# Wenyuan-Vincent-Li/Tensorflow-Implementation-of-Triple-GAN

Hardware: AMD Instinct MI355X
Metric: Triple-GAN train images/sec (G+C+D step) CIFAR-10 32x32 bs=100 (higher is better)
Workload: dtype f32; 1 GPU; CIFAR-10 32x32x3, 4000 labelled, bs=100 fp32 (B_G/L_C/U_C/L_D/U_D=100/50/50/20/80), Good_GAN_cifar10 D+G+C step; global_batch=100, parallelism=dp1, exec_mode=auto, exec_mode_chosen=plan, hip_graph=False

## Files before the change

### include/tg_kernels.h

```cpp
#ifndef TG_KERNELS_H
#define TG_KERNELS_H

#include <stdint.h>

#ifdef __cplusplus
extern "C" {
#endif

typedef enum tg_status {
  TG_OK = 0,
  TG_ERR_INVALID = -1,
  TG_ERR_HIP = -2,
  TG_ERR_STATE = -3
} tg_status;

enum { TG_ACT_NONE = 0, TG_ACT_LRELU = 1, TG_ACT_RELU = 2, TG_ACT_TANH = 3, TG_ACT_SIGMOID = 4, TG_ACT_SOFTPLUS = 5 };

int tg_version(void);
const char* tg_last_error_string(void);
int tg_device_count(void);

int tg_graph_begin_capture(void* stream);
int tg_graph_end_capture(void* stream, void** graph_exec_out);
int tg_graph_launch(void* graph_exec, void* stream);
// ... 125 lines not shown
  int64_t tr_sb, tr_st;
  int32_t t, a, b, a_pad, b_pad;
} tg_prep_job;
int tg_filter_prep_multi_f32(const tg_prep_job* jobs, int n_jobs, void* stream);
typedef struct tg_wn_job {
  const float* slab;
  float* dw;
  const float* v;
  const float* g;
  float* dv;
  float* dg;
  float* coef;
  int32_t n_split, t, c_pad, n_pad, c_in, c_out;
} tg_wn_job;
int tg_filter_grad_tail_multi_f32(const tg_wn_job* jobs, int n_jobs, void* stream);
int tg_slab_reduce_f32(const float* slab, int n_split, int t, int c_pad, int n_pad, int c_dim, int n_dim, float* dst, void* stream);

int tg_wn_bwd_f32(const float* dw, const float* v, const float* g, int rows, int c, float* dv, float* dg, float* coef, void* stream);

int64_t tg_colstats_workspace_floats(int rows, int nseg, int c);
int tg_colstats_f32(int mode, const float* a, int ld_a, const float* b, int ld_b, int rows, int c, const int32_t* seg_rows, int nseg, int act,
                    float alpha, float* workspace, float* s1, float* s2, void* stream);
int tg_seg_scale_shift_act_f32(const float* x, int ld_x, float* y, int ld_y, int rows, int c, int c_zero_to, const int32_t* seg_rows, int nseg,
                               const float* scale, const float* shift, int act, float alpha, void* stream);
int64_t tg_wn_init_workspace_floats(int rows, int c);
int tg_wn_init_f32(const float* t, int ld_t, int rows, int c, int c_zero_to, float eps, float init_scale, int act, float alpha,
                   float* workspace, float* g, float* b, float* y, int ld_y, void* stream);
int tg_seg_actgrad_shift_f32(const float* dy, int ld_dy, const float* yact, int ld_y, float* dx, int ld_dx, int rows, int c,
                             const int32_t* seg_rows, int nseg, const float* shift, int act, float alpha, void* stream);
int tg_mobn_finalize_f32(const float* sums, const int32_t* seg_rows, int nseg, int rows, int c, const float* b, float* pop_mean, float decay,
// ... 169 lines not shown
```

### tensorflow-implementation-of-triple-gan_amd/Model/Good_GAN_cifar10.py

```python
import math
import os

import numpy as np

from Model import model_base
from Model import nn
from tg import grad_penalty, ops
from tg.runtime import ParamStore, ctx


def _he_trunc_normal(rng, shape):
    fan_in = shape[-2] * int(np.prod(shape[:-2])) if len(shape) > 2 else shape[0]
    x = rng.standard_normal(shape)
    bad = np.abs(x) > 2
    while bad.any():
        x[bad] = rng.standard_normal(int(bad.sum()))
        bad = np.abs(x) > 2
    return (x * np.sqrt(1.3 * 2.0 / fan_in)).astype(np.float32)


C_CONVS = [
    ('conv1_1', 128, 'SAME', False), ('conv1_2', 128, 'SAME', False), ('conv1_3', 128, 'SAME', True),
    ('conv2_1', 256, 'SAME', False), ('conv2_2', 256, 'SAME', False), ('conv2_3', 256, 'SAME', True), ('conv3', 512, 'VALID', False)]
D_CONVS = [
# ... 191 lines not shown
        with cx.rng_scoped(cx.phase + '/D'):
            dp, dl = self.discriminator(ximg, yall)
        n_p = x_l_d.n + x_u_d.n
        cut = lambda a: [a.view_rows(0, n_p), a.view_rows(n_p, n_p + G.n), a.view_rows(n_p + G.n, a.n)]
        (p_real, p_fake, p_unl), (l_real, l_fake, l_unl) = cut(dp), cut(dl)
        return [G, [p_real, l_real, p_fake, l_fake, p_unl, l_unl], [C_real, C_unl, C_unl_d, C_fake, C_rep]]


def _dense_view(a):
    assert a.ld == a.c, "layer width must be a multiple of 32 here"
    return a


def _onehot_act(logits, k):
    from tg.runtime import Act
    return Act(ops.argmax_onehot(logits, k), logits.n, 1, 1, k, k)



ZCA_EPS = 1e-5
ZCA_DATA = ('cifar10', 'cifar100')
ZCA_CHUNK = 16384
ZCA_N_MAX = math.isqrt((2 ** 63 - 1) >> 14)


def zca_prefix(config):
    return "cifar100" if getattr(config, 'DATA_NAME', None) == "cifar100" else "cifar10"


def zca_paths(config):
    pre = os.path.join(config.DATA_DIR, zca_prefix(config))
# ... 153 lines not shown
```

### tensorflow-implementation-of-triple-gan_amd/Model/nn.py

```python
import numpy as np

from tg import ops
from tg.runtime import ctx


def int_shape(x):
    return [x.n, x.h, x.w, x.c] if (x.h, x.w) != (1, 1) else [x.n, x.c]


def get_name(layer_name, counters):
    if layer_name not in counters:
        counters[layer_name] = 0
    name = layer_name + '_' + str(counters[layer_name])
    counters[layer_name] += 1
    return name


def _normal(std, seed_key):
    def init(shape):
        cx = ctx()
        cx.init_rng = getattr(cx, 'init_rng', None) or np.random.default_rng(20190430)
        return (cx.init_rng.standard_normal(shape) * std).astype(np.float32)
    return init

# ... 58 lines not shown
    g = cx.get_variable('g', (num_out,), 1.0) if use_weight_normalization else None
    trains = cx.trains()
    gr = (lambda leaf: cx.var_grad(leaf)) if trains else (lambda leaf: None)
    a = _tg_act(nonlinearity)
    fuse = dict(act=a[0], alpha=a[1]) if a else {}
    if use_weight_normalization and init and cx.assign_init:
        return _data_init(cx, x, V, g, b, num_out, k, stride, pad, init_eps, init_scale, nonlinearity)
    if use_weight_normalization and init:
        ones = cx.ws('const:ones', max(num_out, 1024))
        ops.fill(ones, 1.0)
        with cx.no_record():
            y = ops.conv2d(x, V, None, num_out, k, stride, pad, wn=(ones, None))
            y = ops.moments_normalize(y, init_eps, init_scale)
            return _apply_nonlinearity(y, nonlinearity)
    if use_weight_normalization and use_mean_only_batch_normalization:
        if a is None and nonlinearity is not None:
            y = ops.conv2d(x, V, None, num_out, k, stride, pad, wn=(g, gr('g')), mobn=(b, gr('b'), pop), segments=segments,
                           train=not deterministic, kernel_grad=gr('V'))
            return nonlinearity(y)
        return ops.conv2d(x, V, None, num_out, k, stride, pad, wn=(g, gr('g')), mobn=(b, gr('b'), pop), segments=segments,
                          train=not deterministic, kernel_grad=gr('V'), pool=then_pool, **fuse)
    if use_weight_normalization:
        y = ops.conv2d(x, V, b, num_out, k, stride, pad, wn=(g, gr('g')), kernel_grad=gr('V'), bias_grad=gr('b'), **fuse)
        return y if (a or nonlinearity is None) else nonlinearity(y)
    if use_batch_normalization:
        y = ops.conv2d(x, V, None, num_out, k, stride, pad, kernel_grad=gr('V'))
        y = batch_norm_impl(y, is_conv_out=k > 1, deterministic=deterministic)
        return _apply_nonlinearity(y, nonlinearity)
    y = ops.conv2d(x, V, b, num_out, k, stride, pad, kernel_grad=gr('V'), bias_grad=gr('b'), **fuse)
    return y if (a or nonlinearity is None) else nonlinearity(y)
# ... 88 lines not shown
```

### tensorflow-implementation-of-triple-gan_amd/Training/Train_goodGAN.py

```python
import contextlib
import math
import os
import time

import numpy as np
import torch

from config import Config
from Training.options import (LOSSES, NETS, NUM_CLASSES_RANGE, OPTIMIZERS, check_act_dtype, check_clip_norm, check_eval_ema, check_loss,
                              check_mfma_dtype, check_num_classes, check_optimizer, check_sample_metrics, check_wn_init, check_zca, cla_lr, opt, resolve)
from Training.train_base import Train_base, clip_workspace_floats
from tg import dist as tgdist
from tg import executor, lib, ops
from tg.batching import concat_acts
from tg.runtime import Act, Context, PhiloxRNG, ctx, set_context


class Train(Train_base):
    def __init__(self, config, log_dir, save_dir, **kwargs):
        super(Train, self).__init__()
        self.config = config
        self.save_dir = save_dir
        self.log_dir = log_dir
        self.comments = kwargs.get('comments', '')
        o = self.options = resolve(config)
        self.world, self.rank, self.local_rank = tgdist.init()
        try:
            self.cx = ctx()
# ... 125 lines not shown
            g_replay = []
            wgan = self.loss_kind == 'WGAN_GP'
            with cx.wgrad_on_side():
                with cx.sub_tape(('good_generator',), replay=g_replay) as g_tape:
                    G = m.good_generator(self.z_g_ph, self.y_g_ph)
                if wgan:
                    xp = concat_acts([m.as_image(self.x_l_d_ph), m.as_image(self.x_u_d_ph)])
                    self._gp_w, self._gp_grad = m.discriminator_gradient_penalty(xp, m.as_image(G), self.y_g_ph, self.GP_WEIGHT, in_step=True)
            self._g_saved = (G, g_tape, g_replay)
            xz = concat_acts([m.as_image(self.x_u_c_ph), m.as_image(self.x_u_d_ph)])
            if m.zca() is not None:
                xz = m.zca().apply(xz)
            with cx.rng_scoped('D/C'):
                c_logits, _ = m.classifier(xz, True, segments=[c.BATCH_SIZE_U_C, c.BATCH_SIZE_U_D])
            cx.join_wgrad_side()
            oh = ops.argmax_onehot(c_logits, c.NUM_CLASSES)
            self._d_logits = c_logits
            if self._label_override.get('D') is not None:
                oh.copy_(self._label_override['D'])
            k = c.NUM_CLASSES
            oh_unl = Act(oh[:c.BATCH_SIZE_U_C * k], c.BATCH_SIZE_U_C, 1, 1, k, k)
            oh_unl_d = Act(oh[c.BATCH_SIZE_U_C * k:], c.BATCH_SIZE_U_D, 1, 1, k, k)
            self._d_labels = (oh_unl, oh_unl_d)
            ximg = concat_acts([m.as_image(a) for a in (self.x_l_d_ph, self.x_u_d_ph, G, self.x_u_c_ph)])
            yall = concat_acts([self.y_l_d_ph, oh_unl_d, self.y_g_ph, oh_unl])
            with cx.rng_scoped('D/D'):
                _, d_logits = m.discriminator(ximg, yall, want_prob=False)
            if wgan:
                self._wgan_d_head(d_logits, c.BATCH_SIZE_L_D + c.BATCH_SIZE_U_D, c.BATCH_SIZE_G, c.BATCH_SIZE_U_C, self.hyper[2:4], self._gp_w,
                                  self.loss_dev[0:1])
            else:
# ... 29 lines not shown
            G = m.good_generator(self.z_g_ph, self.y_g_ph)
            parts = [self.x_l_c_ph, self.x_u_c_ph] + ([self.x_u_c_ph] if rep else []) + [G]
            segs = [p.n for p in parts]
            xc = concat_acts([m.as_image(p) for p in parts])
            if m.zca() is not None:
                xc = m.zca().apply(xc)
            with cx.rng_scoped('C/C'):
                c_logits, _ = m.classifier(xc, True, segments=segs)
            c_unl = c_logits.view_rows(segs[0], segs[0] + segs[1])
            if self.loss_kind == 'WGAN_GP':
                self._c_logits = c_unl
                self._wgan_c_head(c_logits, segs[0], sum(segs[1:-1]), G.n, self.y_l_c_ph, self.y_g_ph, self.hyper[2:4], self.loss_dev[2:3])
                self._keep_rest('C', cx.backward(stop_at_boundary='classifier' if split else False))
                return
            k = c.NUM_CLASSES
            oh_c = ops.argmax_onehot(c_unl, k)
            self._c_logits = c_unl
            if self._label_override.get('C') is not None:
                oh_c.copy_(self._label_override['C'])
            oh_unl = Act(oh_c, c_unl.n, 1, 1, k, k)
            with cx.rng_scoped('C/D'):
                _, d_unl = m.discriminator(self.x_u_c_ph, oh_unl, want_prob=False)
            self._c_loss(c_logits, segs[0], segs[1], segs[1] if rep else 0, G.n, self.y_l_c_ph, self.y_g_ph, d_unl,
                         self.hyper[2:4], self.loss_dev[2:3])
            self._keep_rest('C', cx.backward(stop_at_boundary='classifier' if split else False))

    def _keep_rest(self, phase, rest):
        self._rest[phase] = (rest, self.cx.counter)

    def _backward_rest(self, phase, net, split):
        rest, counter = self._rest[phase]
# ... 598 lines not shown
```

### tensorflow-implementation-of-triple-gan_amd/csrc/prep.hip

```cpp
#include "tg_common.h"
#include "tg_device.h"

namespace {

__global__ void __launch_bounds__(1024) wn_scale(const float* __restrict__ v, const float* __restrict__ g, int r, int c, float* __restrict__ scale) {
  const int tx = threadIdx.x & 31, ry = threadIdx.x >> 5;
  const int col = blockIdx.x * 32 + tx;
  float a0 = 0.f, a1 = 0.f, a2 = 0.f, a3 = 0.f;
  if (col < c) {
    int i = ry;
    for (; i + 96 < r; i += 128) {
      const float t0 = v[(int64_t)i * c + col], t1 = v[(int64_t)(i + 32) * c + col], t2 = v[(int64_t)(i + 64) * c + col],
                  t3 = v[(int64_t)(i + 96) * c + col];
      a0 += t0 * t0; a1 += t1 * t1; a2 += t2 * t2; a3 += t3 * t3;
    }
    for (; i < r; i += 32) { const float t = v[(int64_t)i * c + col]; a0 += t * t; }
  }
  float acc = (a0 + a1) + (a2 + a3);
  __shared__ float red[32][33];
  red[ry][tx] = acc;
  __syncthreads();
  if (ry == 0 && col < c) {
    for (int k = 1; k < 32; ++k) acc += red[k][tx];
    scale[col] = g[col] * rsqrtf(fmaxf(acc, 1e-12f));
// ... 92 lines not shown
      if (scale) v *= scale[b];
    }
    tile[i][tx] = v;
    if (J.dst_same && a < J.a_pad && b < J.b_pad) J.dst_same[((int64_t)t * J.a_pad + a) * J.b_pad + b] = v;
  }
  __syncthreads();
  if (J.dst_tr) {
    for (int i = ty; i < 32; i += 8) {
      const int b = b0 + i, a = a0 + tx;
      if (b < J.b_pad && a < J.a_pad) J.dst_tr[(int64_t)b * J.tr_sb + (int64_t)t * J.tr_st + a] = tile[tx][i];
    }
  }
}

constexpr int MAX_WN_JOBS = 16;
struct WnJobs { tg_wn_job j[MAX_WN_JOBS]; };

__global__ void __launch_bounds__(256) slab_reduce_multi(WnJobs js) {
  const tg_wn_job& J = js.j[blockIdx.y];
  const int64_t total = (int64_t)J.t * J.c_in * J.c_out;
  const int64_t sstride = (int64_t)J.t * J.c_pad * J.n_pad;
  if ((J.c_out & 3) == 0 && (J.n_pad & 3) == 0 && ((reinterpret_cast<uintptr_t>(J.slab) | reinterpret_cast<uintptr_t>(J.dw)) & 15) == 0) {
    const int64_t total4 = total >> 2;
    const int q = J.c_out >> 2;
    for (int64_t i = (int64_t)blockIdx.x * blockDim.x + threadIdx.x; i < total4; i += (int64_t)gridDim.x * blockDim.x) {
      const int n4 = (int)(i % q);
      const int64_t tc = i / q;
      const int c = (int)(tc % J.c_in), t = (int)(tc / J.c_in);
      const float* p = J.slab + ((int64_t)t * J.c_pad + c) * J.n_pad + 4 * n4;
      float4 acc = make_float4(0.f, 0.f, 0.f, 0.f);
      for (int s = 0; s < J.n_split; ++s) {
        const float4 v = *reinterpret_cast<const float4*>(p + s * sstride);
        acc.x += v.x; acc.y += v.y; acc.z += v.z; acc.w += v.w;
      }
      *reinterpret_cast<float4*>(J.dw + 4 * i) = acc;
    }
    return;
  }
  for (int64_t i = (int64_t)blockIdx.x * blockDim.x + threadIdx.x; i < total; i += (int64_t)gridDim.x * blockDim.x) {
    const int n = (int)(i % J.c_out);
    const int64_t tc = i / J.c_out;
    const int c = (int)(tc % J.c_in), t = (int)(tc / J.c_in);
    const float* p = J.slab + ((int64_t)t * J.c_pad + c) * J.n_pad + n;
    float acc = 0.f;
    for (int s = 0; s < J.n_split; ++s) acc += p[s * sstride];
    J.dw[i] = acc;
  }
}

__global__ void __launch_bounds__(1024) wn_bwd_cols_multi(WnJobs js) {
  const tg_wn_job& J = js.j[blockIdx.y];
  if (J.v == nullptr) return;
  const int r = J.t * J.c_in, c = J.c_out;
  if (blockIdx.x * 32 >= c) return;
  const int tx = threadIdx.x & 31, ry = threadIdx.x >> 5;
  const int col = blockIdx.x * 32 + tx;
  float d0 = 0.f, s0 = 0.f;
  if (col < c) {
    for (int i = ry; i < r; i += 32) {
      const float t = J.v[(int64_t)i * c + col];
      d0 += J.dw[(int64_t)i * c + col] * t;
      s0 += t * t;
    }
  }
  __shared__ float red[2][32][33];
  red[0][ry][tx] = d0;
  red[1][ry][tx] = s0;
  __syncthreads();
  if (ry == 0 && col < c) {
    float dot = d0, ss = s0;
    for (int k = 1; k < 32; ++k) { dot += red[0][k][tx]; ss += red[1][k][tx]; }
    const float nrm = sqrtf(ss);
    J.dg[col] = dot / nrm;
    J.coef[col] = J.g[col] / nrm;
    J.coef[c + col] = dot / ss;
  }
}

__global__ void __launch_bounds__(256) wn_bwd_apply_multi(WnJobs js) {
  const tg_wn_job& J = js.j[blockIdx.y];
  if (J.v == nullptr) return;
  const int c = J.c_out;
  const int64_t n = (int64_t)J.t * J.c_in * c;
  for (int64_t i = (int64_t)blockIdx.x * blockDim.x + threadIdx.x; i < n; i += (int64_t)gridDim.x * blockDim.x) {
    const int col = (int)(i % c);
    J.dv[i] = J.coef[col] * (J.dw[i] - J.v[i] * J.coef[c + col]);
// ... 196 lines not shown
  js.first_block[n_jobs] = blocks;
  hipStream_t s = tg::as_stream(stream);
  tg::ProfScope prof(tg::PC_PREP, 0, bytes, s);
  if (any_wn) {
    hipLaunchKernelGGL(wn_scale_multi, dim3((max_b + 31) / 32, n_jobs), dim3(1024), 0, s, js);
    TG_CHECK_LAUNCH("wn_scale_multi");
  }
  hipLaunchKernelGGL(filter_prep_multi, dim3(blocks), dim3(256), 0, s, js);
  TG_CHECK_LAUNCH("filter_prep_multi");
  return TG_OK;
}

int tg_filter_grad_tail_multi_f32(const tg_wn_job* jobs, int n_jobs, void* stream) {
  TG_REQUIRE(jobs && n_jobs >= 1 && n_jobs <= MAX_WN_JOBS, "filter_grad_tail_multi: n_jobs=%d out of range", n_jobs);
  WnJobs js;
  int64_t max_total = 0;
  int max_c = 0;
  bool any_wn = false;
  double bytes = 0;
  for (int i = 0; i < n_jobs; ++i) {
    const tg_wn_job& j = jobs[i];
    TG_REQUIRE(j.slab && j.dw && j.n_split >= 1 && j.t >= 1 && j.c_in >= 1 && j.c_out >= 1 && j.c_in <= j.c_pad && j.c_out <= j.n_pad,
               "filter_grad_tail_multi: job %d has bad geometry", i);
    TG_REQUIRE(j.v == nullptr || (j.g && j.dv && j.dg && j.coef), "filter_grad_tail_multi: job %d lacks weight-norm buffers", i);
    js.j[i] = j;
    const int64_t total = (int64_t)j.t * j.c_in * j.c_out;
    max_total = total > max_total ? total : max_total;
    max_c = j.c_out > max_c ? j.c_out : max_c;
    any_wn = any_wn || j.v != nullptr;
    bytes += 4.0 * total * (j.n_split + 1 + (j.v ? 5 : 0));
  }
  hipStream_t s = tg::as_stream(stream);
  tg::ProfScope prof(tg::PC_PREP, 0, bytes, s);
  int gx = (int)((max_total + 255) / 256);
  gx = gx > 1024 ? 1024 : gx;
  hipLaunchKernelGGL(slab_reduce_multi, dim3(gx, n_jobs), dim3(256), 0, s, js);
  TG_CHECK_LAUNCH("slab_reduce_multi");
  if (any_wn) {
    hipLaunchKernelGGL(wn_bwd_cols_multi, dim3((max_c + 31) / 32, n_jobs), dim3(1024), 0, s, js);
    TG_CHECK_LAUNCH("wn_bwd_cols_multi");
    hipLaunchKernelGGL(wn_bwd_apply_multi, dim3(gx, n_jobs), dim3(256), 0, s, js);
    TG_CHECK_LAUNCH("wn_bwd_apply_multi");
  }
  return TG_OK;
}

int tg_slab_reduce_f32(const float* slab, int n_split, int t, int c_pad, int n_pad, int c, int n, float* dst, void* stream) {
  TG_REQUIRE(slab && dst && n_split >= 1 && c <= c_pad && n <= n_pad, "slab_reduce: bad args");
  hipStream_t s = tg::as_stream(stream);
  tg::ProfScope prof(tg::PC_PREP, 0, 4.0 * t * c * n * (n_split + 1), s);
  const int64_t total = (int64_t)t * c * n;
  if (n_split >= 32 && total <= 65536)
    hipLaunchKernelGGL(slab_reduce_wide, dim3((unsigned)((total + 31) / 32)), dim3(256), 0, s, slab, n_split, t, c_pad, n_pad, c, n, dst);
  else
// ... 37 lines not shown
```

### tensorflow-implementation-of-triple-gan_amd/tg/lib.py

```python
import ctypes as C
import os
import re

_HERE = os.path.dirname(os.path.abspath(__file__))
LIB_PATH = os.path.join(os.path.dirname(_HERE), "csrc", os.environ.get("TG_LIB", "libtg_hip.so"))

TG_MAX_TAPS = 25
ACT = {None: 0, 'none': 0, 'lrelu': 1, 'relu': 2, 'tanh': 3, 'sigmoid': 4, 'softplus': 5}


class IgemmDesc(C.Structure):
    _fields_ = [
        ("n_img", C.c_int32),
        ("h_in", C.c_int32), ("w_in", C.c_int32), ("ld_in", C.c_int32),
        ("h_v", C.c_int32), ("w_v", C.c_int32),
        ("s_y", C.c_int32), ("s_x", C.c_int32),
        ("h_out", C.c_int32), ("w_out", C.c_int32), ("ld_out", C.c_int32),
        ("os_y", C.c_int32), ("os_x", C.c_int32), ("oo_y", C.c_int32), ("oo_x", C.c_int32),
        ("c_out", C.c_int32), ("n_store", C.c_int32), ("n_taps", C.c_int32),
        ("dy", C.c_int8 * TG_MAX_TAPS), ("dx", C.c_int8 * TG_MAX_TAPS),
        ("tapw", C.c_int16 * TG_MAX_TAPS),
        ("w_sn", C.c_int64), ("w_st", C.c_int64),
        ("act", C.c_int32), ("alpha", C.c_float),
        ("n_group", C.c_int32),
# ... 14 lines not shown

class CopyJob(C.Structure):
    _fields_ = [("src", C.c_void_p), ("dst", C.c_void_p), ("n", C.c_int64)]


class RngJob(C.Structure):
    _fields_ = [("out", C.c_void_p), ("n", C.c_int64), ("mode", C.c_int32), ("a", C.c_float), ("b", C.c_float), ("stream_id", C.c_uint32)]


HEADER_PATH = os.path.join(os.path.dirname(os.path.dirname(_HERE)), "include", "tg_kernels.h")

_SCALARS = {"int": C.c_int, "int32_t": C.c_int32, "int64_t": C.c_int64, "uint32_t": C.c_uint32, "float": C.c_float}
_RET = {"int": C.c_int, "int64_t": C.c_int64, "const char*": C.c_char_p}
_NOCHECK = {"tg_version", "tg_last_error_string", "tg_device_count", "tg_prof_num_classes", "tg_prof_class_name",
            "tg_colstats_workspace_floats", "tg_wn_init_workspace_floats", "tg_igemm_colsum_supported", "tg_conv3x3_policy", "tg_conv3x3_launches",
            "tg_deconv5x5s2_narrow_supported", "tg_conv3x3_packed_supported"}
_NEGATIVE_IS_ERROR = {"tg_wgrad_splits", "tg_wgrad_splits_bf16", "tg_wgrad_workspace_bytes", "tg_filter_workspace_bytes",
                      "tg_igemm_workspace_bytes", "tg_deconv5x5s2_narrow_wgrad_workspace_bytes",
                      "tg_conv3x3_packed_wgrad_workspace_bytes", "tg_grad_norm_workspace_bytes",
                      "tg_tf_histogram_workspace_bytes", "tg_feature_moments_workspace_bytes"}
HOST_INT_ARRAYS = {"seg_rows", "tapmap"}


def _ctype_of(decl):
    decl = re.sub(r"/\*.*?\*/", "", decl).strip()
    name = decl.split()[-1].lstrip("*")
    typ = decl[: decl.rindex(name)].strip()
    if typ.endswith("*"):
        base = typ.replace("const", "").replace("*", "").strip()
        if base == "tg_igemm_desc":
            return C.c_void_p if name == "descs" else C.POINTER(IgemmDesc)
# ... 103 lines not shown
```

Before: 7219 images/sec.

## Fuse classifier dense mean-only-BN head with argmax onehot into single-workgroup kernels

```diff
diff --git a/include/tg_kernels.h b/include/tg_kernels.h
--- a/include/tg_kernels.h
+++ b/include/tg_kernels.h
@@ -163,6 +163,14 @@
   int32_t n_split, t, c_pad, n_pad, c_in, c_out;
 } tg_wn_job;
 int tg_filter_grad_tail_multi_f32(const tg_wn_job* jobs, int n_jobs, void* stream);
+int tg_dense_mobn_head_supported(int rows, int c_in, int k, int nseg);
+int tg_dense_mobn_head_dw_parts(void);
+int tg_dense_mobn_head_fwd_f32(const float* x, int ld_x, const float* w, int ld_w, const float* b, float* pop_mean, float decay,
+                               const int32_t* seg_rows, int nseg, int rows, int c_in, int k, float* t, float* y, int ld_out, float* means,
+                               float* onehot, void* stream);
+int tg_dense_mobn_head_bwd_f32(const float* gy, int ld_gy, const float* x, int ld_x, const float* w, int ld_w, const int32_t* seg_rows, int nseg,
+                               int rows, int c_in, int k, float* db, float* dt, float* dx, int ld_dx, float* dw_slabs, int c_pad, int n_pad,
+                               void* stream);
 int tg_slab_reduce_f32(const float* slab, int n_split, int t, int c_pad, int n_pad, int c_dim, int n_dim, float* dst, void* stream);
 
 int tg_wn_bwd_f32(const float* dw, const float* v, const float* g, int rows, int c, float* dv, float* dg, float* coef, void* stream);
diff --git a/tensorflow-implementation-of-triple-gan_amd/Model/Good_GAN_cifar10.py b/tensorflow-implementation-of-triple-gan_amd/Model/Good_GAN_cifar10.py
--- a/tensorflow-implementation-of-triple-gan_amd/Model/Good_GAN_cifar10.py
+++ b/tensorflow-implementation-of-triple-gan_amd/Model/Good_GAN_cifar10.py
@@ -5,7 +5,7 @@
 
 from Model import model_base
 from Model import nn
-from tg import grad_penalty, ops
+from tg import grad_penalty, heads, ops
 from tg.runtime import ParamStore, ctx
 
 
@@ -229,7 +229,7 @@
 
 def _onehot_act(logits, k):
     from tg.runtime import Act
-    return Act(ops.argmax_onehot(logits, k), logits.n, 1, 1, k, k)
+    return Act(heads.argmax_onehot(logits, k), logits.n, 1, 1, k, k)
 
 
 
diff --git a/tensorflow-implementation-of-triple-gan_amd/Model/nn.py b/tensorflow-implementation-of-triple-gan_amd/Model/nn.py
--- a/tensorflow-implementation-of-triple-gan_amd/Model/nn.py
+++ b/tensorflow-implementation-of-triple-gan_amd/Model/nn.py
@@ -1,6 +1,6 @@
 import numpy as np
 
-from tg import ops
+from tg import heads, ops
 from tg.runtime import ctx
 
 
@@ -96,6 +96,8 @@
             y = ops.moments_normalize(y, init_eps, init_scale)
             return _apply_nonlinearity(y, nonlinearity)
     if use_weight_normalization and use_mean_only_batch_normalization:
+        if then_pool is None and heads.eligible(cx, x, num_out, k, segments, not deterministic, nonlinearity, init):
+            return heads.dense_mobn_head(x, V, g, b, pop, num_out, segments, gr('V'), gr('g'), gr('b'))
         if a is None and nonlinearity is not None:
             y = ops.conv2d(x, V, None, num_out, k, stride, pad, wn=(g, gr('g')), mobn=(b, gr('b'), pop), segments=segments,
                            train=not deterministic, kernel_grad=gr('V'))
diff --git a/tensorflow-implementation-of-triple-gan_amd/Training/Train_goodGAN.py b/tensorflow-implementation-of-triple-gan_amd/Training/Train_goodGAN.py
--- a/tensorflow-implementation-of-triple-gan_amd/Training/Train_goodGAN.py
+++ b/tensorflow-implementation-of-triple-gan_amd/Training/Train_goodGAN.py
@@ -11,7 +11,7 @@
                               check_mfma_dtype, check_num_classes, check_optimizer, check_sample_metrics, check_wn_init, check_zca, cla_lr, opt, resolve)
 from Training.train_base import Train_base, clip_workspace_floats
 from tg import dist as tgdist
-from tg import executor, lib, ops
+from tg import executor, heads, lib, ops
 from tg.batching import concat_acts
 from tg.runtime import Act, Context, PhiloxRNG, ctx, set_context
 
@@ -167,7 +167,7 @@
             with cx.rng_scoped('D/C'):
                 c_logits, _ = m.classifier(xz, True, segments=[c.BATCH_SIZE_U_C, c.BATCH_SIZE_U_D])
             cx.join_wgrad_side()
-            oh = ops.argmax_onehot(c_logits, c.NUM_CLASSES)
+            oh = heads.argmax_onehot(c_logits, c.NUM_CLASSES)
             self._d_logits = c_logits
             if self._label_override.get('D') is not None:
                 oh.copy_(self._label_override['D'])
@@ -227,7 +227,7 @@
                 self._keep_rest('C', cx.backward(stop_at_boundary='classifier' if split else False))
                 return
             k = c.NUM_CLASSES
-            oh_c = ops.argmax_onehot(c_unl, k)
+            oh_c = heads.argmax_onehot(c_unl, k)
             self._c_logits = c_unl
             if self._label_override.get('C') is not None:
                 oh_c.copy_(self._label_override['C'])
diff --git a/tensorflow-implementation-of-triple-gan_amd/csrc/head.hip b/tensorflow-implementation-of-triple-gan_amd/csrc/head.hip
--- /dev/null
+++ b/tensorflow-implementation-of-triple-gan_amd/csrc/head.hip
@@ -0,0 +1,259 @@
+#include "tg_common.h"
+#include "tg_device.h"
+
+namespace {
+
+constexpr int HEAD_MAX_ROWS = 1024;
+constexpr int HEAD_MAX_CIN = 256;
+constexpr int HEAD_MAX_K = 32;
+constexpr int HEAD_MAX_SEG = 8;
+constexpr int HEAD_DW_PARTS = 4;
+
+struct HeadSegs { int nseg; int rows[HEAD_MAX_SEG]; };
+
+__device__ __forceinline__ void load_filter(float (*ws)[32], const float* __restrict__ w, int ld_w, int c_in, int k) {
+  for (int i = threadIdx.x; i < c_in * 32; i += 1024) {
+    const int c = i >> 5, j = i & 31;
+    ws[c][j] = j < k ? w[(int64_t)c * ld_w + j] : 0.f;
+  }
+}
+
+__device__ __forceinline__ float seg_colsum(const float* a, int ld, int r0, int r1, int k, float (*red)[33]) {
+  const int j = threadIdx.x & 31, rr = threadIdx.x >> 5;
+  float part = 0.f;
+  if (j < k)
+    for (int r = r0 + rr; r < r1; r += 32) part += a[(int64_t)r * ld + j];
+  __syncthreads();
+  red[rr][j] = part;
+  __syncthreads();
+  float tot = 0.f;
+  if (rr == 0) {
+    tot = red[0][j];
+    for (int q = 1; q < 32; ++q) tot += red[q][j];
+  }
+  return tot;
+}
+
+__global__ void __launch_bounds__(1024) dense_mobn_head_fwd(const float* __restrict__ x, int ld_x, const float* __restrict__ w, int ld_w,
+                                                            const float* __restrict__ b, float* __restrict__ pop, float decay, HeadSegs st,
+                                                            int rows, int c_in, int k, float* t_out, float* y, int ld_out,
+                                                            float* __restrict__ means, float* __restrict__ onehot) {
+  __shared__ __attribute__((aligned(16))) float ws[HEAD_MAX_CIN][32];
+  __shared__ float red[32][33];
+  __shared__ float shift[HEAD_MAX_SEG][32];
+  load_filter(ws, w, ld_w, c_in, k);
+  __syncthreads();
+  const int wave = threadIdx.x >> 6, lane = threadIdx.x & 63;
+  const int ngrp = (k + 7) >> 3, nblk = (rows + 63) >> 6;
+  for (int task = wave; task < nblk * ngrp; task += 16) {
+    const int blk = task / ngrp, j0 = (task - blk * ngrp) * 8;
+    const int r = blk * 64 + lane;
+    if (r >= rows) continue;
+    const float* xr = x + (int64_t)r * ld_x;
+    float acc[8] = {0.f, 0.f, 0.f, 0.f, 0.f, 0.f, 0.f, 0.f};
+#pragma unroll 4
+    for (int c = 0; c < c_in; c += 4) {
+      const float4 xv = *reinterpret_cast<const float4*>(xr + c);
+      const float xs[4] = {xv.x, xv.y, xv.z, xv.w};
+#pragma unroll
+      for (int u = 0; u < 4; ++u) {
+        const float4 w0 = *reinterpret_cast<const float4*>(&ws[c + u][j0]), w1 = *reinterpret_cast<const float4*>(&ws[c + u][j0 + 4]);
+        acc[0] = fmaf(xs[u], w0.x, acc[0]); acc[1] = fmaf(xs[u], w0.y, acc[1]); acc[2] = fmaf(xs[u], w0.z, acc[2]); acc[3] = fmaf(xs[u], w0.w, acc[3]);
+        acc[4] = fmaf(xs[u], w1.x, acc[4]); acc[5] = fmaf(xs[u], w1.y, acc[5]); acc[6] = fmaf(xs[u], w1.z, acc[6]); acc[7] = fmaf(xs[u], w1.w, acc[7]);
+      }
+    }
+#pragma unroll
+    for (int u = 0; u < 8; ++u)
+      if (j0 + u < k) {
+        y[(int64_t)r * ld_out + j0 + u] = acc[u];
+        if (t_out) t_out[(int64_t)r * ld_out + j0 + u] = acc[u];
+      }
+  }
+  __threadfence_block();
+  __syncthreads();
+  const int j = threadIdx.x & 31, rr = threadIdx.x >> 5;
+  float pm = 0.f, bb = 0.f;
+  if (rr == 0 && j < k) { pm = pop[j]; bb = b ? b[j] : 0.f; }
+  int r0 = 0;
+  for (int s = 0; s < st.nseg; ++s) {
+    const float tot = seg_colsum(y, ld_out, r0, r0 + st.rows[s], k, red);
+    if (rr == 0 && j < k) {
+      const float m = tot / (float)st.rows[s];
+      means[s * k + j] = m;
+      shift[s][j] = bb - m;
+      pm = pm * decay + m * (1.f - decay);
+    }
+    r0 += st.rows[s];
+  }
+  if (rr == 0 && j < k) pop[j] = pm;
+  __syncthreads();
+  r0 = 0;
+  for (int s = 0; s < st.nseg; ++s) {
+    const int r1 = r0 + st.rows[s];
+    const float sh = j < k ? shift[s][j] : 0.f;
+    for (int base = r0; base < r1; base += 32) {
+      const int r = base + rr;
+      const bool live = r < r1;
+      float v = 0.f;
+      if (live && j < k) v = y[(int64_t)r * ld_out + j] + sh;
+      if (live && j < ld_out) y[(int64_t)r * ld_out + j] = v;
+      if (onehot) {
+        float m = j < k ? v : -INFINITY;
+        int am = j;
+#pragma unroll
+        for (int o = 16; o > 0; o >>= 1) {
+          const float om = __shfl_xor(m, o, 32);
+          const int oa = __shfl_xor(am, o, 32);
+          if (om > m || (om == m && oa < am)) { m = om; am = oa; }
+        }
+        if (live && j < k) onehot[(int64_t)r * k + j] = j == am ? 1.f : 0.f;
+      }
+    }
+    r0 = r1;
+  }
+}
+
+__global__ void __launch_bounds__(1024) dense_mobn_head_bwd(const float* __restrict__ gy, int ld_gy, const float* __restrict__ x, int ld_x,
+                                                            const float* __restrict__ w, int ld_w, HeadSegs st, int rows, int c_in, int k,
+                                                            float* __restrict__ db, float* dt, float* __restrict__ dx, int ld_dx,
+                                                            float* __restrict__ dw_slabs, int c_pad, int n_pad) {
+  __shared__ __attribute__((aligned(16))) float ws[HEAD_MAX_CIN][32];
+  __shared__ float red[32][33];
+  __shared__ float shift[HEAD_MAX_SEG][32];
+  load_filter(ws, w, ld_w, c_in, k);
+  const int j = threadIdx.x & 31, rr = threadIdx.x >> 5;
+  float tot = 0.f;
+  int r0 = 0;
+  for (int s = 0; s < st.nseg; ++s) {
+    const float v = seg_colsum(gy, ld_gy, r0, r0 + st.rows[s], k, red);
+    if (rr == 0 && j < k) {
+      shift[s][j] = -v / (float)st.rows[s];
+      tot += v;
+    }
+    r0 += st.rows[s];
+  }
+  if (rr == 0 && j < k) db[j] = tot;
+  __syncthreads();
+  r0 = 0;
+  for (int s = 0; s < st.nseg; ++s) {
+    const int r1 = r0 + st.rows[s];
+    const float sh = j < k ? shift[s][j] : 0.f;
+    for (int r = r0 + rr; r < r1; r += 32) dt[(int64_t)r * 32 + j] = j < k ? gy[(int64_t)r * ld_gy + j] + sh : 0.f;
+    r0 = r1;
+  }
+  __threadfence_block();
+  __syncthreads();
+  const int wave = threadIdx.x >> 6, lane = threadIdx.x & 63;
+  const int nblk = (rows + 63) >> 6, k4 = (k + 3) >> 2;
+  const int cq = (c_in + 3) >> 2, per = (cq + 3) >> 2;
+  for (int task = wave; task < nblk * 4; task += 16) {
+    const int blk = task >> 2, q0 = (task & 3) * per, q1 = min(cq, q0 + per);
+    const int r = blk * 64 + lane;
+    if (r >= rows) continue;
+    float d[HEAD_MAX_K];
+#pragma unroll
+    for (int q = 0; q < 8; ++q) {
+      float4 v = make_float4(0.f, 0.f, 0.f, 0.f);
+      if (q < k4) v = *reinterpret_cast<const float4*>(dt + (int64_t)r * 32 + 4 * q);
+      d[4 * q] = v.x; d[4 * q + 1] = v.y; d[4 * q + 2] = v.z; d[4 * q + 3] = v.w;
+    }
+    for (int q = q0; q < q1; ++q) {
+      float o[4];
+#pragma unroll
+      for (int u = 0; u < 4; ++u) {
+        float a = 0.f;
+#pragma unroll
+        for (int p = 0; p < 8; ++p)
+          if (p < k4) {
+            const float4 wv = *reinterpret_cast<const float4*>(&ws[4 * q + u][4 * p]);
+            a = fmaf(d[4 * p], wv.x, a); a = fmaf(d[4 * p + 1], wv.y, a); a = fmaf(d[4 * p + 2], wv.z, a); a = fmaf(d[4 * p + 3], wv.w, a);
+          }
+        o[u] = a;
+      }
+      *reinterpret_cast<float4*>(dx + (int64_t)r * ld_dx + 4 * q) = make_float4(o[0], o[1], o[2], o[3]);
+    }
+  }
+  const int ngrp = (k + 7) >> 3, ncb = (c_in + 63) >> 6;
+  const int rper = (rows + HEAD_DW_PARTS - 1) / HEAD_DW_PARTS;
+  for (int task = wave; task < ncb * ngrp * HEAD_DW_PARTS; task += 16) {
+    const int part = task % HEAD_DW_PARTS, rest = task / HEAD_DW_PARTS;
+    const int cb = rest / ngrp, j0 = (rest - cb * ngrp) * 8;
+    const int c = cb * 64 + lane;
+    if (c >= c_in) continue;
+    const int ra = part * rper, rb = min(rows, ra + rper);
+    float acc[8] = {0.f, 0.f, 0.f, 0.f, 0.f, 0.f, 0.f, 0.f};
+#pragma unroll 8
+    for (int r = ra; r < rb; ++r) {
+      const float xv = x[(int64_t)r * ld_x + c];
+      const float4 d0 = *reinterpret_cast<const float4*>(dt + (int64_t)r * 32 + j0), d1 = *reinterpret_cast<const float4*>(dt + (int64_t)r * 32 + j0 + 4);
+      acc[0] = fmaf(xv, d0.x, acc[0]); acc[1] = fmaf(xv, d0.y, acc[1]); acc[2] = fmaf(xv, d0.z, acc[2]); acc[3] = fmaf(xv, d0.w, acc[3]);
+      acc[4] = fmaf(xv, d1.x, acc[4]); acc[5] = fmaf(xv, d1.y, acc[5]); acc[6] = fmaf(xv, d1.z, acc[6]); acc[7] = fmaf(xv, d1.w, acc[7]);
+    }
+    float* o = dw_slabs + ((int64_t)part * c_pad + c) * n_pad + j0;
+#pragma unroll
+    for (int u = 0; u < 8; ++u)
+      if (j0 + u < k) o[u] = acc[u];
+  }
+}
+
+int make_head_segs(HeadSegs& st, const int32_t* seg_rows, int nseg, int rows) {
+  TG_REQUIRE(seg_rows && nseg >= 1 && nseg <= HEAD_MAX_SEG, "dense_mobn_head: nseg=%d out of range", nseg);
+  int tot = 0;
+  st.nseg = nseg;
+  for (int i = 0; i < nseg; ++i) { st.rows[i] = seg_rows[i]; tot += seg_rows[i]; TG_REQUIRE(seg_rows[i] > 0, "dense_mobn_head: empty segment %d", i); }
+  TG_REQUIRE(tot == rows, "dense_mobn_head: segments sum to %d, rows=%d", tot, rows);
+  return TG_OK;
+}
+
+bool aligned16(const void* p) { return (reinterpret_cast<uintptr_t>(p) & 15) == 0; }
+
+}
+
+extern "C" {
+
+int tg_dense_mobn_head_supported(int rows, int c_in, int k, int nseg) {
+  return rows >= 1 && rows <= HEAD_MAX_ROWS && c_in >= 4 && c_in <= HEAD_MAX_CIN && c_in % 4 == 0 && k >= 1 && k <= HEAD_MAX_K && nseg >= 1 &&
+         nseg <= HEAD_MAX_SEG;
+}
+
+int tg_dense_mobn_head_dw_parts(void) { return HEAD_DW_PARTS; }
+
+int tg_dense_mobn_head_fwd_f32(const float* x, int ld_x, const float* w, int ld_w, const float* b, float* pop_mean, float decay,
+                               const int32_t* seg_rows, int nseg, int rows, int c_in, int k, float* t, float* y, int ld_out, float* means,
+                               float* onehot, void* stream) {
+  TG_REQUIRE(x && w && pop_mean && y && means, "dense_mobn_head_fwd: null buffer");
+  TG_REQUIRE(tg_dense_mobn_head_supported(rows, c_in, k, nseg), "dense_mobn_head_fwd: rows=%d c_in=%d k=%d nseg=%d outside one workgroup's bounds",
+             rows, c_in, k, nseg);
+  TG_REQUIRE(ld_x >= c_in && ld_x % 4 == 0 && aligned16(x) && ld_w >= k && ld_out >= k && ld_out <= 32,
+             "dense_mobn_head_fwd: ld_x=%d ld_w=%d ld_out=%d", ld_x, ld_w, ld_out);
+  HeadSegs st;
+  int rc = make_head_segs(st, seg_rows, nseg, rows);
+  if (rc != TG_OK) return rc;
+  hipStream_t s = tg::as_stream(stream);
+  tg::ProfScope prof(tg::PC_NORM, 2.0 * rows * c_in * k, 4.0 * (rows * (c_in + 2.0 * k) + c_in * k), s);
+  hipLaunchKernelGGL(dense_mobn_head_fwd, dim3(1), dim3(1024), 0, s, x, ld_x, w, ld_w, b, pop_mean, decay, st, rows, c_in, k, t, y, ld_out, means,
+                     onehot);
+  TG_CHECK_LAUNCH("dense_mobn_head_fwd");
+  return TG_OK;
+}
+
+int tg_dense_mobn_head_bwd_f32(const float* gy, int ld_gy, const float* x, int ld_x, const float* w, int ld_w, const int32_t* seg_rows, int nseg,
+                               int rows, int c_in, int k, float* db, float* dt, float* dx, int ld_dx, float* dw_slabs, int c_pad, int n_pad,
+                               void* stream) {
+  TG_REQUIRE(gy && x && w && db && dt && dx && dw_slabs, "dense_mobn_head_bwd: null buffer");
+  TG_REQUIRE(tg_dense_mobn_head_supported(rows, c_in, k, nseg), "dense_mobn_head_bwd: rows=%d c_in=%d k=%d nseg=%d outside one workgroup's bounds",
+             rows, c_in, k, nseg);
+  TG_REQUIRE(ld_gy >= k && ld_x >= c_in && ld_w >= k && ld_dx >= c_in && ld_dx % 4 == 0 && aligned16(dx) && aligned16(dt) && c_pad >= c_in && n_pad >= k,
+             "dense_mobn_head_bwd: ld_gy=%d ld_x=%d ld_w=%d ld_dx=%d c_pad=%d n_pad=%d", ld_gy, ld_x, ld_w, ld_dx, c_pad, n_pad);
+  HeadSegs st;
+  int rc = make_head_segs(st, seg_rows, nseg, rows);
+  if (rc != TG_OK) return rc;
+  hipStream_t s = tg::as_stream(stream);
+  tg::ProfScope prof(tg::PC_NORM, 4.0 * rows * c_in * k, 4.0 * (rows * (2.0 * c_in + 2.0 * k) + 2.0 * c_in * k), s);
+  hipLaunchKernelGGL(dense_mobn_head_bwd, dim3(1), dim3(1024), 0, s, gy, ld_gy, x, ld_x, w, ld_w, st, rows, c_in, k, db, dt, dx, ld_dx, dw_slabs,
+                     c_pad, n_pad);
+  TG_CHECK_LAUNCH("dense_mobn_head_bwd");
+  return TG_OK;
+}
+
+}
diff --git a/tensorflow-implementation-of-triple-gan_amd/csrc/prep.hip b/tensorflow-implementation-of-triple-gan_amd/csrc/prep.hip
--- a/tensorflow-implementation-of-triple-gan_amd/csrc/prep.hip
+++ b/tensorflow-implementation-of-triple-gan_amd/csrc/prep.hip
@@ -130,62 +130,123 @@
 }
 
 constexpr int MAX_WN_JOBS = 16;
-struct WnJobs { tg_wn_job j[MAX_WN_JOBS]; };
+struct WnJobs {
+  tg_wn_job j[MAX_WN_JOBS];
+  int first_slab[MAX_WN_JOBS + 1], first_cols[MAX_WN_JOBS + 1];
+  int n;
+  unsigned slab_vec, cols_vec;
+};
+
+__device__ __forceinline__ int job_of_block(const int* first, int n, int blk) {
+  int job = 0;
+  while (job + 1 < n && blk >= first[job + 1]) ++job;
+  return job;
+}
+
+template <typename T> __device__ __forceinline__ void add_to(T& a, const T& v);
+template <> __device__ __forceinline__ void add_to<float>(float& a, const float& v) { a += v; }
+template <> __device__ __forceinline__ void add_to<float4>(float4& a, const float4& v) { a.x += v.x; a.y += v.y; a.z += v.z; a.w += v.w; }
+
+template <typename T, int N> __device__ __forceinline__ void slab_batch(T& acc, const float* p, int64_t sstride) {
+  T v[N];
+#pragma unroll
+  for (int k = 0; k < N; ++k) v[k] = *reinterpret_cast<const T*>(p + k * sstride);
+#pragma unroll
+  for (int k = 0; k < N; ++k) add_to(acc, v[k]);
+}
+
+template <typename T> __device__ __forceinline__ T slab_sum(const float* p, int n_split, int64_t sstride) {
+  T acc;
+  __builtin_memset(&acc, 0, sizeof(T));
+  int s = 0;
+  for (; s + 8 <= n_split; s += 8) slab_batch<T, 8>(acc, p + s * sstride, sstride);
+  if (s + 4 <= n_split) { slab_batch<T, 4>(acc, p + s * sstride, sstride); s += 4; }
+  if (s + 2 <= n_split) { slab_batch<T, 2>(acc, p + s * sstride, sstride); s += 2; }
+  if (s < n_split) slab_batch<T, 1>(acc, p + s * sstride, sstride);
+  return acc;
+}
 
 __global__ void __launch_bounds__(256) slab_reduce_multi(WnJobs js) {
-  const tg_wn_job& J = js.j[blockIdx.y];
+  const int job = job_of_block(js.first_slab, js.n, blockIdx.x);
+  const tg_wn_job& J = js.j[job];
   const int64_t total = (int64_t)J.t * J.c_in * J.c_out;
   const int64_t sstride = (int64_t)J.t * J.c_pad * J.n_pad;
-  if ((J.c_out & 3) == 0 && (J.n_pad & 3) == 0 && ((reinterpret_cast<uintptr_t>(J.slab) | reinterpret_cast<uintptr_t>(J.dw)) & 15) == 0) {
-    const int64_t total4 = total >> 2;
+  const int64_t i = (int64_t)(blockIdx.x - js.first_slab[job]) * 256 + threadIdx.x;
+  if ((js.slab_vec >> job) & 1u) {
+    if (i >= (total >> 2)) return;
     const int q = J.c_out >> 2;
-    for (int64_t i = (int64_t)blockIdx.x * blockDim.x + threadIdx.x; i < total4; i += (int64_t)gridDim.x * blockDim.x) {
-      const int n4 = (int)(i % q);
-      const int64_t tc = i / q;
-      const int c = (int)(tc % J.c_in), t = (int)(tc / J.c_in);
-      const float* p = J.slab + ((int64_t)t * J.c_pad + c) * J.n_pad + 4 * n4;
-      float4 acc = make_float4(0.f, 0.f, 0.f, 0.f);
-      for (int s = 0; s < J.n_split; ++s) {
-        const float4 v = *reinterpret_cast<const float4*>(p + s * sstride);
-        acc.x += v.x; acc.y += v.y; acc.z += v.z; acc.w += v.w;
+    const int n4 = (int)(i % q);
+    const int64_t tc = i / q;
+    const int c = (int)(tc % J.c_in), t = (int)(tc / J.c_in);
+    const float* p = J.slab + ((int64_t)t * J.c_pad + c) * J.n_pad + 4 * n4;
+    *reinterpret_cast<float4*>(J.dw + 4 * i) = slab_sum<float4>(p, J.n_split, sstride);
+    return;
+  }
+  if (i >= total) return;
+  const int n = (int)(i % J.c_out);
+  const int64_t tc = i / J.c_out;
+  const int c = (int)(tc % J.c_in), t = (int)(tc / J.c_in);
+  J.dw[i] = slab_sum<float>(J.slab + ((int64_t)t * J.c_pad + c) * J.n_pad + n, J.n_split, sstride);
+}
+
+__global__ void __launch_bounds__(1024) wn_bwd_cols_multi(WnJobs js) {
+  __shared__ float red[2][256][17];
+  const int job = job_of_block(js.first_cols, js.n, blockIdx.x);
+  const tg_wn_job& J = js.j[job];
+  const int grp = blockIdx.x - js.first_cols[job];
+  const int r = J.t * J.c_in, c = J.c_out;
+  float dot = 0.f, ss = 0.f;
+  int col;
+  bool lead;
+  if ((js.cols_vec >> job) & 1u) {
+    const int tx = threadIdx.x & 3, ry = threadIdx.x >> 2;
+    const int col0 = grp * 16 + tx * 4;
+    float4 d = make_float4(0.f, 0.f, 0.f, 0.f), s = d;
+    if (col0 < c) {
+#pragma unroll 2
+      for (int i = ry; i < r; i += 256) {
+        const float4 t = *reinterpret_cast<const float4*>(J.v + (int64_t)i * c + col0);
+        const float4 w = *reinterpret_cast<const float4*>(J.dw + (int64_t)i * c + col0);
+        d.x += w.x * t.x; d.y += w.y * t.y; d.z += w.z * t.z; d.w += w.w * t.w;
+        s.x += t.x * t.x; s.y += t.y * t.y; s.z += t.z * t.z; s.w += t.w * t.w;
       }
-      *reinterpret_cast<float4*>(J.dw + 4 * i) = acc;
-    }
-    return;
-  }
-  for (int64_t i = (int64_t)blockIdx.x * blockDim.x + threadIdx.x; i < total; i += (int64_t)gridDim.x * blockDim.x) {
-    const int n = (int)(i % J.c_out);
-    const int64_t tc = i / J.c_out;
-    const int c = (int)(tc % J.c_in), t = (int)(tc / J.c_in);
-    const float* p = J.slab + ((int64_t)t * J.c_pad + c) * J.n_pad + n;
-    float acc = 0.f;
-    for (int s = 0; s < J.n_split; ++s) acc += p[s * sstride];
-    J.dw[i] = acc;
-  }
-}
-
-__global__ void __launch_bounds__(1024) wn_bwd_cols_multi(WnJobs js) {
-  const tg_wn_job& J = js.j[blockIdx.y];
-  if (J.v == nullptr) return;
-  const int r = J.t * J.c_in, c = J.c_out;
-  if (blockIdx.x * 32 >= c) return;
-  const int tx = threadIdx.x & 31, ry = threadIdx.x >> 5;
-  const int col = blockIdx.x * 32 + tx;
-  float d0 = 0.f, s0 = 0.f;
-  if (col < c) {
-    for (int i = ry; i < r; i += 32) {
-      const float t = J.v[(int64_t)i * c + col];
-      d0 += J.dw[(int64_t)i * c + col] * t;
-      s0 += t * t;
-    }
-  }
-  __shared__ float red[2][32][33];
-  red[0][ry][tx] = d0;
-  red[1][ry][tx] = s0;
-  __syncthreads();
-  if (ry == 0 && col < c) {
-    float dot = d0, ss = s0;
-    for (int k = 1; k < 32; ++k) { dot += red[0][k][tx]; ss += red[1][k][tx]; }
+    }
+    red[0][ry][tx * 4 + 0] = d.x; red[0][ry][tx * 4 + 1] = d.y; red[0][ry][tx * 4 + 2] = d.z; red[0][ry][tx * 4 + 3] = d.w;
+    red[1][ry][tx * 4 + 0] = s.x; red[1][ry][tx * 4 + 1] = s.y; red[1][ry][tx * 4 + 2] = s.z; red[1][ry][tx * 4 + 3] = s.w;
+    __syncthreads();
+    const int cx = threadIdx.x & 15, k = threadIdx.x >> 4;
+    if (k < 16) {
+      dot = red[0][k][cx]; ss = red[1][k][cx];
+      for (int m = 1; m < 16; ++m) { dot += red[0][k + 16 * m][cx]; ss += red[1][k + 16 * m][cx]; }
+    }
+    __syncthreads();
+    if (k < 16) { red[0][k][cx] = dot; red[1][k][cx] = ss; }
+    __syncthreads();
+    col = grp * 16 + cx;
+    lead = k == 0 && col < c;
+    if (lead)
+      for (int m = 1; m < 16; ++m) { dot += red[0][m][cx]; ss += red[1][m][cx]; }
+  } else {
+    float(*rd)[32][33] = reinterpret_cast<float(*)[32][33]>(&red[0][0][0]);
+    float(*rs)[32][33] = reinterpret_cast<float(*)[32][33]>(&red[1][0][0]);
+    const int tx = threadIdx.x & 31, ry = threadIdx.x >> 5;
+    col = grp * 32 + tx;
+    if (col < c) {
+#pragma unroll 4
+      for (int i = ry; i < r; i += 32) {
+        const float t = J.v[(int64_t)i * c + col];
+        dot += J.dw[(int64_t)i * c + col] * t;
+        ss += t * t;
+      }
+    }
+    (*rd)[ry][tx] = dot;
+    (*rs)[ry][tx] = ss;
+    __syncthreads();
+    lead = ry == 0 && col < c;
+    if (lead)
+      for (int k = 1; k < 32; ++k) { dot += (*rd)[k][tx]; ss += (*rs)[k][tx]; }
+  }
+  if (lead) {
     const float nrm = sqrtf(ss);
     J.dg[col] = dot / nrm;
     J.coef[col] = J.g[col] / nrm;
@@ -412,9 +473,10 @@
 int tg_filter_grad_tail_multi_f32(const tg_wn_job* jobs, int n_jobs, void* stream) {
   TG_REQUIRE(jobs && n_jobs >= 1 && n_jobs <= MAX_WN_JOBS, "filter_grad_tail_multi: n_jobs=%d out of range", n_jobs);
   WnJobs js;
-  int64_t max_total = 0;
-  int max_c = 0;
-  bool any_wn = false;
+  js.n = n_jobs;
+  js.slab_vec = js.cols_vec = 0;
+  int64_t max_total = 0, slab_blocks = 0;
+  int cols_blocks = 0;
   double bytes = 0;
   for (int i = 0; i < n_jobs; ++i) {
     const tg_wn_job& j = jobs[i];
@@ -424,18 +486,28 @@
     js.j[i] = j;
     const int64_t total = (int64_t)j.t * j.c_in * j.c_out;
     max_total = total > max_total ? total : max_total;
-    max_c = j.c_out > max_c ? j.c_out : max_c;
-    any_wn = any_wn || j.v != nullptr;
+    const bool quad = (j.c_out & 3) == 0;
+    const bool svec = quad && (j.n_pad & 3) == 0 && ((reinterpret_cast<uintptr_t>(j.slab) | reinterpret_cast<uintptr_t>(j.dw)) & 15) == 0;
+    const bool cvec = quad && j.v && ((reinterpret_cast<uintptr_t>(j.v) | reinterpret_cast<uintptr_t>(j.dw)) & 15) == 0;
+    js.slab_vec |= (unsigned)svec << i;
+    js.cols_vec |= (unsigned)cvec << i;
+    js.first_slab[i] = (int)slab_blocks;
+    js.first_cols[i] = cols_blocks;
+    slab_blocks += ((svec ? total >> 2 : total) + 255) / 256;
+    cols_blocks += j.v ? (cvec ? (j.c_out + 15) / 16 : (j.c_out + 31) / 32) : 0;
+    TG_REQUIRE(slab_blocks < (1 << 30), "filter_grad_tail_multi: job %d makes the launch too large", i);
     bytes += 4.0 * total * (j.n_split + 1 + (j.v ? 5 : 0));
   }
+  js.first_slab[n_jobs] = (int)slab_blocks;
+  js.first_cols[n_jobs] = cols_blocks;
   hipStream_t s = tg::as_stream(stream);
   tg::ProfScope prof(tg::PC_PREP, 0, bytes, s);
-  int gx = (int)((max_total + 255) / 256);
-  gx = gx > 1024 ? 1024 : gx;
-  hipLaunchKernelGGL(slab_reduce_multi, dim3(gx, n_jobs), dim3(256), 0, s, js);
+  hipLaunchKernelGGL(slab_reduce_multi, dim3((unsigned)slab_blocks), dim3(256), 0, s, js);
   TG_CHECK_LAUNCH("slab_reduce_multi");
-  if (any_wn) {
-    hipLaunchKernelGGL(wn_bwd_cols_multi, dim3((max_c + 31) / 32, n_jobs), dim3(1024), 0, s, js);
+  if (cols_blocks) {
+    int gx = (int)((max_total + 255) / 256);
+    gx = gx > 1024 ? 1024 : gx;
+    hipLaunchKernelGGL(wn_bwd_cols_multi, dim3(cols_blocks), dim3(1024), 0, s, js);
     TG_CHECK_LAUNCH("wn_bwd_cols_multi");
     hipLaunchKernelGGL(wn_bwd_apply_multi, dim3(gx, n_jobs), dim3(256), 0, s, js);
     TG_CHECK_LAUNCH("wn_bwd_apply_multi");
diff --git a/tensorflow-implementation-of-triple-gan_amd/tg/heads.py b/tensorflow-implementation-of-triple-gan_amd/tg/heads.py
--- /dev/null
+++ b/tensorflow-implementation-of-triple-gan_amd/tg/heads.py
@@ -0,0 +1,67 @@
+from . import lib, ops
+from .runtime import ctx, pad32, seg_array
+
+FWD, BWD = 'tg_dense_mobn_head_fwd_f32', 'tg_dense_mobn_head_bwd_f32'
+
+
+def eligible(cx, x, num_out, k, segments, train, nonlinearity, init):
+    if k != 1 or x.h != 1 or x.w != 1:
+        return False
+    cx.head_onehot = None
+    if not train or init or nonlinearity is not None or cx.mfma_dtype == 'bf16' or x.dtype != 'f32' or num_out > 32:
+        return False
+    if cx.store_of(cx.scope_name('V')).read_ema:
+        return False
+    nseg = 1 if segments is None else len(segments)
+    return bool(lib.call('tg_dense_mobn_head_supported', x.rows, x.c, num_out, nseg))
+
+
+def dense_mobn_head(x, V, g, b, pop, num_out, segments, kernel_grad, g_grad, b_grad, decay=0.9):
+    cx = ctx()
+    ops.require_f32(x, 'dense_mobn_head')
+    c_in, co_p, rows = x.c, pad32(num_out), x.rows
+    seg_rows = ops._segs(x, segments)
+    needs_w = cx.trains() and kernel_grad is not None
+    needs_x = cx.tape is not None and x.requires_grad
+    _, _, w_hwio = ops._prepared_filter(cx, V, g, 1, c_in, num_out, x.ld, co_p, True)
+    y = cx.new_act(x.n, 1, 1, num_out, co_p, requires_grad=needs_w or needs_x)
+    y.strided_grad_ok = True
+    means = cx.scratch('hmean', len(seg_rows) * num_out)
+    onehot = cx.scratch('oh', rows * num_out)
+    lib.call(FWD, x.ptr, x.ld, ops._p(w_hwio), co_p, ops._p(b), ops._p(pop), decay, seg_array(seg_rows), len(seg_rows), rows, c_in, num_out,
+             None, y.ptr, y.ld, ops._p(means), ops._p(onehot), cx.stream)
+    cx.head_onehot = (cx.phase, y.t.data_ptr(), rows, y.ld, num_out, onehot)
+    if not (needs_w or needs_x):
+        return y
+
+    def bwd():
+        gy = y.grad
+        assert gy is not None, "dense_mobn_head backward: no gradient reached the logits"
+        ops._single_consumer(y, gy)
+        parts = lib.call('tg_dense_mobn_head_dw_parts')
+        db = b_grad if needs_w else cx.scratch('db', num_out)
+        dt = cx.scratch('hdt', rows * 32)
+        slab = cx.scratch('slab', parts * x.ld * co_p)
+        gx = cx.grad_of(x) if needs_x else None
+        dx = gx.t if needs_x else cx.scratch('hdx', rows * x.ld)
+        lib.call(BWD, gy.ptr, gy.ld, x.ptr, x.ld, ops._p(w_hwio), co_p, seg_array(seg_rows), len(seg_rows), rows, c_in, num_out, ops._p(db),
+                 ops._p(dt), ops._p(dx), x.ld, ops._p(slab), x.ld, co_p, cx.stream)
+        if needs_w:
+            dw = cx.scratch('dw', c_in * num_out)
+            coef = cx.scratch('coef', 2 * num_out)
+            cx.tail_jobs.append(lib.WnJob(slab.data_ptr(), dw.data_ptr(), V.data_ptr(), g.data_ptr(), kernel_grad.data_ptr(), g_grad.data_ptr(),
+                                          coef.data_ptr(), parts, 1, x.ld, co_p, c_in, num_out))
+
+    cx.record(bwd)
+    return y
+
+
+def argmax_onehot(logits, k):
+    cx = ctx()
+    rec = getattr(cx, 'head_onehot', None)
+    if rec is not None and rec[0] == cx.phase and rec[4] == k and rec[3] == logits.ld and logits.h == 1 and logits.w == 1 and logits.c == k:
+        off, per = logits.t.data_ptr() - rec[1], 4 * logits.ld
+        if off >= 0 and off % per == 0 and off // per + logits.n <= rec[2]:
+            r0 = off // per
+            return rec[5][r0 * k:(r0 + logits.n) * k]
+    return ops.argmax_onehot(logits, k)
diff --git a/tensorflow-implementation-of-triple-gan_amd/tg/lib.py b/tensorflow-implementation-of-triple-gan_amd/tg/lib.py
--- a/tensorflow-implementation-of-triple-gan_amd/tg/lib.py
+++ b/tensorflow-implementation-of-triple-gan_amd/tg/lib.py
@@ -52,7 +52,7 @@
 _RET = {"int": C.c_int, "int64_t": C.c_int64, "const char*": C.c_char_p}
 _NOCHECK = {"tg_version", "tg_last_error_string", "tg_device_count", "tg_prof_num_classes", "tg_prof_class_name",
             "tg_colstats_workspace_floats", "tg_wn_init_workspace_floats", "tg_igemm_colsum_supported", "tg_conv3x3_policy", "tg_conv3x3_launches",
-            "tg_deconv5x5s2_narrow_supported", "tg_conv3x3_packed_supported"}
+            "tg_deconv5x5s2_narrow_supported", "tg_conv3x3_packed_supported", "tg_dense_mobn_head_supported", "tg_dense_mobn_head_dw_parts"}
 _NEGATIVE_IS_ERROR = {"tg_wgrad_splits", "tg_wgrad_splits_bf16", "tg_wgrad_workspace_bytes", "tg_filter_workspace_bytes",
                       "tg_igemm_workspace_bytes", "tg_deconv5x5s2_narrow_wgrad_workspace_bytes",
                       "tg_conv3x3_packed_wgrad_workspace_bytes", "tg_grad_norm_workspace_bytes",
```

Result: no change. 7254 images/sec (median of 6 runs) (+0.5%).
